# NVlabs/FoundationPose

Hardware: NVIDIA H100
Metric: pose-hypotheses/sec at 640x480 RGB-D, 252 hyp, 5 refine iters (higher is better)
Workload: dtype f16

## Files before the change

foundationpose_b200/csrc/fp_gemm.cu:

```cuda
#include "fp_gemm.cuh"

#include <stdarg.h>
#include <stdlib.h>
#include <string.h>

#include <mutex>
#include <vector>

#include "fp_common.cuh"
#include "fp_wgmma.cuh"

namespace fp {

static std::atomic<unsigned long long> g_launch_count{0};
static thread_local bool t_capturing = false;
void note_launches(int n) {
  if (!t_capturing) g_launch_count.fetch_add((unsigned long long)n, std::memory_order_relaxed);
}
unsigned long long launch_count() { return g_launch_count.load(std::memory_order_relaxed); }
void set_capturing(bool on) { t_capturing = on; }

std::atomic<bool> g_prof_on{false};
static std::mutex g_prof_mu;

struct ProfRec {
  cudaEvent_t e0, e1;
  double work;
  int kind;
};
static std::vector<ProfRec> g_prof_recs;

void prof_mark_begin(int kind, double work, cudaStream_t stream) {
  if (!g_prof_on) return;
  ProfRec r;
  r.kind = kind;
  r.work = work;
  cudaEventCreate(&r.e0);
  cudaEventCreate(&r.e1);
  cudaEventRecord(r.e0, stream);
  std::lock_guard<std::mutex> lk(g_prof_mu);
  g_prof_recs.push_back(r);
}
void prof_mark_end(cudaStream_t stream) {
  if (!g_prof_on) return;
  std::lock_guard<std::mutex> lk(g_prof_mu);
  if (g_prof_recs.empty()) return;
  cudaEventRecord(g_prof_recs.back().e1, stream);
}
int prof_collect(int kind, double* total_ms, double* total_work, int* launches) {
  FP_CUDA_OK(cudaDeviceSynchronize());
  std::lock_guard<std::mutex> lk(g_prof_mu);
  double ms = 0, work = 0;
  int n = 0;
  std::vector<ProfRec> keep;
  for (auto& r : g_prof_recs) {
    if (r.kind != kind) {
      keep.push_back(r);
      continue;
    }
    float t = 0.f;
    cudaEventElapsedTime(&t, r.e0, r.e1);
    ms += t;
    work += r.work;
    ++n;
    cudaEventDestroy(r.e0);
    cudaEventDestroy(r.e1);
  }
  g_prof_recs.swap(keep);
  *total_ms = ms;
  *total_work = work;
  *launches = n;
  return 0;
}

static thread_local char t_last_error[1024] = "";
void set_last_error(const char* fmt, ...) {
  va_list ap;
  va_start(ap, fmt);
  vsnprintf(t_last_error, sizeof(t_last_error), fmt, ap);
  va_end(ap);
}
const char* get_last_error() { return t_last_error; }

static thread_local int t_pdl_skip = 0;
void pdl_skip_next() { t_pdl_skip = 1; }

bool pdl_enabled() {
  if (t_pdl_skip) {
    t_pdl_skip = 0;
    return false;
  }
  static int on = -1;
  if (on < 0) {
    const char* e = getenv("FPOSE_PDL");
    on = (e && e[0] == '0') ? 0 : 1;
  }
  return on != 0;
}

struct GemmParams {
  int lg_bw, lg_bh;
  int bw, bh, bn;
  int tiles_w, tiles_h, tiles_n, n_tiles_n, total_tiles;
  int num_kb, chunks_per_tap;
  int dim_w, dim_h, dim_n;
  short tap_off[9][5];
  int Ho, Wo, n_img, Cout;
  const float* bias;
  int has_res;
  int odim_h, odim_n;
  int out_split;
  const float* post_add;
  int relu;
  double alg_flops;
};

constexpr int kBlockM = 128;
constexpr int kBlockK = 64;
constexpr int kABytes = kBlockM * kBlockK * 2;
constexpr int kTileThreads = 384;
constexpr int kSlabBytes = kBlockM * 64 * 2;
constexpr int kSmemOptIn = 232448;

constexpr int kWideSlabs = 2;
constexpr int kWideProducerRegs = 40;
constexpr int kWideConsumerRegs = 232;
template <int BN>
struct TileCfg {
  static constexpr int kBBytes = BN * kBlockK * 2;
  static constexpr int kStageBytes = kABytes + kBBytes;
  static constexpr int kSlabs = BN > 128 ? kWideSlabs : BN / 64;
  static constexpr int kPasses = BN / 64 / kSlabs;
  static constexpr int kStagingBytes = kSlabs * kSlabBytes;
  static constexpr int kRing = kSmemOptIn - kStagingBytes - 1024  - 256 ;
  static constexpr int kStages = (kRing / kStageBytes) > 8 ? 8 : (kRing / kStageBytes);
  static constexpr int kSmemBytes = kStages * kStageBytes + kStagingBytes + 1024 + 256;
  static_assert(kSmemBytes <= kSmemOptIn, "tile configuration exceeds the 227 KB opt-in shared memory");
  static_assert(kPasses * kSlabs * 64 == BN, "the epilogue passes must cover the tile's channels");
};

template <int BN>
__global__ void __launch_bounds__(kTileThreads, 1)
    gemm_tile_kernel(const __grid_constant__ CUtensorMap map_a, const __grid_constant__ CUtensorMap map_b,
                     const __grid_constant__ CUtensorMap map_out, const __grid_constant__ CUtensorMap map_res,
                     const __grid_constant__ GemmParams p) {
  using Cfg = TileCfg<BN>;
  constexpr int S = Cfg::kStages;
  constexpr int NSLAB = Cfg::kSlabs;
  constexpr int JP = BN / 8 / Cfg::kPasses;
  extern __shared__ uint8_t smem_raw[];
  uint8_t* smem = reinterpret_cast<uint8_t*>((reinterpret_cast<uintptr_t>(smem_raw) + 1023) & ~uintptr_t(1023));
  uint8_t* staging = smem + S * Cfg::kStageBytes;
  uint64_t* bars = reinterpret_cast<uint64_t*>(staging + Cfg::kStagingBytes);
  uint64_t* full = bars;
  uint64_t* empty = bars + S;
  uint64_t* res_full = bars + 2 * S;

  const int m_tiles = p.tiles_w * p.tiles_h * p.tiles_n;
  const int total = m_tiles * p.n_tiles_n;

  if (threadIdx.x == 0) {
    tma_prefetch_desc(&map_a);
    tma_prefetch_desc(&map_b);
    tma_prefetch_desc(&map_out);
    if (p.has_res) tma_prefetch_desc(&map_res);
    for (int s = 0; s < S; ++s) {
      mbar_init(&full[s], 1);
      mbar_init(&empty[s], 256);
    }
    mbar_init(res_full, 1);
    mbar_fence_init();
  }
  __syncthreads();
  pdl_trigger();
  pdl_wait();

  auto decode = [&](int t, int& n_tile, int& tw, int& th, int& tn) {
    n_tile = t % p.n_tiles_n;
    const int m_tile = t / p.n_tiles_n;
    tw = m_tile % p.tiles_w;
    th = (m_tile / p.tiles_w) % p.tiles_h;
    tn = m_tile / (p.tiles_w * p.tiles_h);
  };

  if (threadIdx.x < 128) {
    if constexpr (BN > 128) regs_release<kWideProducerRegs>();
    if (threadIdx.x == 0) {
      int stage = 0, phase = 0;
      for (int t = blockIdx.x; t < total; t += gridDim.x) {
        int n_tile, tw, th, tn;
        decode(t, n_tile, tw, th, tn);
        int base[5] = {0, 0, 0, 0, 0};
        base[p.dim_w] += tw * p.bw;
        if (p.dim_h >= 0) base[p.dim_h] += th * p.bh;
        if (p.dim_n >= 0) base[p.dim_n] += tn * p.bn;
        int tap = 0, chunk = 0;
        for (int kb = 0; kb < p.num_kb; ++kb) {
          mbar_wait(&empty[stage], phase ^ 1);
          uint8_t* sa = smem + stage * Cfg::kStageBytes;
          mbar_expect_tx(&full[stage], Cfg::kStageBytes);
          tma_load_5d(&map_a, &full[stage], sa, base[0] + p.tap_off[tap][0] + chunk * kBlockK, base[1] + p.tap_off[tap][1],
                      base[2] + p.tap_off[tap][2], base[3] + p.tap_off[tap][3], base[4] + p.tap_off[tap][4]);
          tma_load_2d(&map_b, &full[stage], sa + kABytes, kb * kBlockK, n_tile * BN);
          if (++chunk == p.chunks_per_tap) {
            chunk = 0;
            ++tap;
          }
          if (++stage == S) {
            stage = 0;
            phase ^= 1;
          }
        }
      }
    }
    return;
  }

  if constexpr (BN > 128) regs_acquire<kWideConsumerRegs>();
  const int ct = threadIdx.x - 128;
  const int cw = ct >> 7;
  const int lane = threadIdx.x & 31;
  const int r0 = 64 * cw + 16 * ((ct >> 5) & 3) + (lane >> 2);
  const int cq = 2 * (lane & 3);
  const bool leader = (ct == 0);
  float acc[BN / 2];
#pragma unroll
  for (int i = 0; i < BN / 2; ++i) acc[i] = 0.f;
  int stage = 0, phase = 0, it = 0;
  for (int t = blockIdx.x; t < total; t += gridDim.x, ++it) {
    int n_tile, tw, th, tn;
    decode(t, n_tile, tw, th, tn);
    const int n0 = tn * p.bn;
    int n_o0 = n0, coff = 0;
    if (p.out_split > 0) {
      n_o0 = n0 % p.out_split;
      coff = (n0 / p.out_split) * p.Cout;
    }
    int oc[5] = {0, 0, 0, 0, 0}, rc[5] = {0, 0, 0, 0, 0};
    oc[1] = rc[1] = tw * p.bw;
    if (p.odim_h >= 0) oc[p.odim_h] = rc[p.odim_h] = th * p.bh;
    if (p.odim_n >= 0) {
      oc[p.odim_n] = n_o0;
      rc[p.odim_n] = n0;
    }
    if (leader) asm volatile("cp.async.bulk.wait_group.read 0;" ::: "memory");
    asm volatile("bar.sync 1, 256;" ::: "memory");
    if (leader && p.has_res) {
      mbar_expect_tx(res_full, NSLAB * kSlabBytes);
      for (int s = 0; s < NSLAB; ++s)
        tma_load_5d(&map_res, res_full, staging + s * kSlabBytes, n_tile * BN + s * 64, rc[1], rc[2], rc[3], rc[4]);
    }

    int prev = -1;
    for (int kb = 0; kb < p.num_kb; ++kb) {
      mbar_wait(&full[stage], phase);
      const uint32_t sa = smem_u32(smem + stage * Cfg::kStageBytes);
      const uint64_t da = gmma_desc_sw128(sa + (uint32_t)cw * 8192u);
      const uint64_t db = gmma_desc_sw128(sa + kABytes);
      wgmma_fence();
#pragma unroll
      for (int k = 0; k < kBlockK / 16; ++k)
        Wgmma<BN>::ss(acc, da + (uint64_t)(2 * k), db + (uint64_t)(2 * k), (kb > 0 || k > 0) ? 1u : 0u);
      wgmma_commit();
      if (prev >= 0) {
        wgmma_wait<1>();
        mbar_arrive(&empty[prev]);
      }
      prev = stage;
      if (++stage == S) {
        stage = 0;
        phase ^= 1;
      }
    }
    wgmma_wait<0>();
    fence_regs(acc);
    if (prev >= 0) mbar_arrive(&empty[prev]);

    const float* bias = p.bias + n_tile * BN;
    const float* pap[2] = {nullptr, nullptr};
    if (p.post_add) {
#pragma unroll
      for (int h = 0; h < 2; ++h) {
        const int row = r0 + 8 * h;
        const int jj = row & (p.bw - 1), ii = (row >> p.lg_bw) & (p.bh - 1);
        const int i = th * p.bh + ii, j = min(tw * p.bw + jj, p.Wo - 1);
        pap[h] = p.post_add + (size_t)(i * p.Wo + j) * p.Cout + n_tile * BN;
      }
    }
#pragma unroll
    for (int ps = 0; ps < Cfg::kPasses; ++ps) {
      const int c0 = n_tile * BN + ps * NSLAB * 64;
      if (ps > 0) {
        if (leader) asm volatile("cp.async.bulk.wait_group.read 0;" ::: "memory");
        asm volatile("bar.sync 1, 256;" ::: "memory");
        if (leader && p.has_res) {
          mbar_expect_tx(res_full, NSLAB * kSlabBytes);
          for (int s = 0; s < NSLAB; ++s)
            tma_load_5d(&map_res, res_full, staging + s * kSlabBytes, c0 + s * 64, rc[1], rc[2], rc[3], rc[4]);
        }
      }
      if (p.has_res) mbar_wait(res_full, (uint32_t)((it * Cfg::kPasses + ps) & 1));
#pragma unroll
      for (int jl = 0; jl < JP; ++jl) {
        const int j = ps * JP + jl;
        const int col = 8 * j + cq;
        const float2 b = __ldg(reinterpret_cast<const float2*>(bias + col));
        uint8_t* slab = staging + (jl >> 3) * kSlabBytes;
#pragma unroll
        for (int h = 0; h < 2; ++h) {
          const int row = r0 + 8 * h;
          uint32_t* cell = reinterpret_cast<uint32_t*>(slab + row * 128 + ((((uint32_t)j & 7u) ^ (uint32_t)(row & 7)) << 4) + cq * 2);
          float a0 = acc[4 * j + 2 * h] + b.x, a1 = acc[4 * j + 2 * h + 1] + b.y;
          if (p.has_res) {
            const float2 r = __half22float2(*reinterpret_cast<const __half2*>(cell));
            a0 += r.x;
            a1 += r.y;
          }
          if (p.relu) {
            a0 = fmaxf(a0, 0.f);
            a1 = fmaxf(a1, 0.f);
          }
          if (pap[h]) {
            const float2 pe = __ldg(reinterpret_cast<const float2*>(pap[h] + col));
            a0 += pe.x;
            a1 += pe.y;
          }
          *cell = pack_half2(a0, a1);
        }
      }
      asm volatile("fence.proxy.async.shared::cta;" ::: "memory");
      asm volatile("bar.sync 1, 256;" ::: "memory");
      if (leader) {
        for (int s = 0; s < NSLAB; ++s)
          tma_store_5d(&map_out, staging + s * kSlabBytes, coff + c0 + s * 64, oc[1], oc[2], oc[3], oc[4]);
        asm volatile("cp.async.bulk.commit_group;" ::: "memory");
      }
    }
  }
  if (leader) asm volatile("cp.async.bulk.wait_group 0;" ::: "memory");
}

static int g_num_sms = 0;

typedef CUresult (*EncodeTiledFn)(CUtensorMap*, CUtensorMapDataType, cuuint32_t, void*, const cuuint64_t*,
                                  const cuuint64_t*, const cuuint32_t*, const cuuint32_t*,
                                  CUtensorMapInterleave, CUtensorMapSwizzle, CUtensorMapL2promotion,
                                  CUtensorMapFloatOOBfill);

static EncodeTiledFn get_encode_fn() {
  static EncodeTiledFn fn = nullptr;
  static std::once_flag once;
  std::call_once(once, [] {
    void* p = nullptr;
    cudaDriverEntryPointQueryResult qres;
    if (cudaGetDriverEntryPoint("cuTensorMapEncodeTiled", &p, cudaEnableDefault, &qres) == cudaSuccess &&
        qres == cudaDriverEntryPointSuccess)
      fn = reinterpret_cast<EncodeTiledFn>(p);
  });
  return fn;
}

static int encode_map(CUtensorMap* map, const void* base, int rank, const uint64_t* dims,
                      const uint64_t* strides_bytes , const uint32_t* box, bool swizzle128 = true) {
  EncodeTiledFn fn = get_encode_fn();
  FP_REQUIRE(fn != nullptr, "cuTensorMapEncodeTiled entry point not available (no CUDA driver?)");
  cuuint64_t gdim[5];
  cuuint64_t gstr[4];
  cuuint32_t bdim[5];
  cuuint32_t estr[5];
  for (int i = 0; i < rank; ++i) {
    gdim[i] = dims[i];
    bdim[i] = box[i];
    estr[i] = 1;
  }
  for (int i = 0; i < rank - 1; ++i) gstr[i] = strides_bytes[i];
  CUresult r = fn(map, CU_TENSOR_MAP_DATA_TYPE_FLOAT16, (cuuint32_t)rank, const_cast<void*>(base), gdim, gstr,
                  bdim, estr, CU_TENSOR_MAP_INTERLEAVE_NONE, swizzle128 ? CU_TENSOR_MAP_SWIZZLE_128B : CU_TENSOR_MAP_SWIZZLE_NONE,
                  CU_TENSOR_MAP_L2_PROMOTION_L2_256B, CU_TENSOR_MAP_FLOAT_OOB_FILL_NONE);
  FP_REQUIRE(r == CUDA_SUCCESS,
             "cuTensorMapEncodeTiled failed (%d): rank %d dims [%llu %llu %llu %llu %llu] box [%u %u %u %u %u]",
             (int)r, rank, (unsigned long long)dims[0], (unsigned long long)(rank > 1 ? dims[1] : 0),
             (unsigned long long)(rank > 2 ? dims[2] : 0), (unsigned long long)(rank > 3 ? dims[3] : 0),
             (unsigned long long)(rank > 4 ? dims[4] : 0), box[0], rank > 1 ? box[1] : 0, rank > 2 ? box[2] : 0,
             rank > 3 ? box[3] : 0, rank > 4 ? box[4] : 0);
  return 0;
}

int encode_map_f16(CUtensorMap* map, const void* base, int rank, const uint64_t* dims, const uint64_t* strides_bytes,
                   const uint32_t* box) {
  return encode_map(map, base, rank, dims, strides_bytes, box);
}
int encode_map_f16_linear(CUtensorMap* map, const void* base, int rank, const uint64_t* dims,
                          const uint64_t* strides_bytes, const uint32_t* box) {
  return encode_map(map, base, rank, dims, strides_bytes, box, false);
}
int num_sms() {
  if (g_num_sms == 0) {
    int dev = 0;
    if (cudaGetDevice(&dev) != cudaSuccess) return 0;
    if (cudaDeviceGetAttribute(&g_num_sms, cudaDevAttrMultiProcessorCount, dev) != cudaSuccess) return 0;
  }
  return g_num_sms;
}

static int ilog2(int v) {
  int l = 0;
  while ((1 << l) < v) ++l;
  return l;
}

template <int BN>
static int launch_bn(const CUtensorMap& ma, const CUtensorMap& mb, const CUtensorMap& mo, const CUtensorMap& mr,
                     const GemmParams& p, cudaStream_t stream) {
  using Cfg = TileCfg<BN>;
  static std::atomic<unsigned long long> attr_mask{0};
  if (!device_bit_test(attr_mask)) {
    FP_CUDA_OK(cudaFuncSetAttribute(gemm_tile_kernel<BN>, cudaFuncAttributeMaxDynamicSharedMemorySize, Cfg::kSmemBytes));
    device_bit_set(attr_mask);
  }
  const int sms = num_sms();
  FP_REQUIRE(sms > 0, "no CUDA device");
  const int grid = p.total_tiles < sms ? p.total_tiles : sms;
  prof_mark_begin(0, p.alg_flops, stream);
  FP_CUDA_OK(launch_pdl(gemm_tile_kernel<BN>, dim3(grid), dim3(kTileThreads), Cfg::kSmemBytes, stream, 1, ma, mb, mo, mr, p));
  prof_mark_end(stream);
  note_launches(1);
  FP_CUDA_OK(cudaGetLastError());
  return 0;
}

int stem_conv_launch(const GemmLayer& L, cudaStream_t stream);

static int gemm_layer_plan(const GemmLayer& L, cudaStream_t stream, int* tile_n) {
  if (L.kind == LK_CONV7_S2) {
    if (tile_n) {
      *tile_n = 64;
      return 0;
    }
    return stem_conv_launch(L, stream);
  }
  GemmParams p;
  memset(&p, 0, sizeof(p));
  CUtensorMap ma, mb;
  const uint64_t E = 2;
  int Ho, Wo, taps, ktot;
  int BN;
  uint64_t dims[5], str[4];
  uint32_t box[5];

  switch (L.kind) {
    case LK_LINEAR: {
      FP_REQUIRE(L.Cin % 64 == 0, "LINEAR: K=%d not a multiple of 64", L.Cin);
      Ho = 1;
      Wo = L.Win;
      taps = 1;
      p.chunks_per_tap = L.Cin / 64;
      p.bw = 128; p.bh = 1; p.bn = 1;
      p.dim_w = 1; p.dim_h = -1; p.dim_n = -1;
      dims[0] = L.Cin; dims[1] = L.Win; dims[2] = 1; dims[3] = 1; dims[4] = 1;
      str[0] = L.Cin * E; str[1] = str[0] * L.Win; str[2] = str[1]; str[3] = str[1];
      box[0] = 64; box[1] = 128; box[2] = 1; box[3] = 1; box[4] = 1;
      p.tiles_w = (L.Win + 127) / 128; p.tiles_h = 1; p.tiles_n = 1;
      break;
    }
    case LK_CONV3_S1: {
      FP_REQUIRE(L.Cin % 64 == 0, "CONV3_S1: Cin=%d not a multiple of 64", L.Cin);
      Ho = L.Hin; Wo = L.Win;
      taps = 9;
      p.chunks_per_tap = L.Cin / 64;
      if (Wo % 8 == 0 && Ho % 8 == 0) { p.bw = 8; p.bh = 8; p.bn = 2; }
      else if (Wo % 4 == 0 && Ho % 4 == 0) { p.bw = 4; p.bh = 4; p.bn = 8; }
      else FP_REQUIRE(false, "CONV3_S1: unsupported spatial size %dx%d", Ho, Wo);
      const uint64_t sw_ = (uint64_t)L.Cin * E, sh_ = sw_ * L.Win, sn_ = sh_ * L.Hin;
      p.dim_w = 1; p.dim_h = 2; p.dim_n = 3;
      dims[0] = L.Cin; dims[1] = L.Win; dims[2] = L.Hin; dims[3] = L.n_img; dims[4] = 1;
      str[0] = sw_; str[1] = sh_; str[2] = sn_; str[3] = sn_ * L.n_img;
      box[0] = 64; box[1] = p.bw; box[2] = p.bh; box[3] = p.bn; box[4] = 1;
      for (int r = 0; r < 3; ++r)
        for (int s = 0; s < 3; ++s) {
          p.tap_off[r * 3 + s][1] = (short)(s - 1);
          p.tap_off[r * 3 + s][2] = (short)(r - 1);
        }
      p.tiles_w = Wo / p.bw; p.tiles_h = Ho / p.bh; p.tiles_n = (L.n_img + p.bn - 1) / p.bn;
      break;
    }
    case LK_CONV3_S2: {
      FP_REQUIRE(L.Cin % 64 == 0, "CONV3_S2: Cin=%d not a multiple of 64", L.Cin);
      FP_REQUIRE(L.Hin % 2 == 0 && L.Win % 2 == 0, "CONV3_S2: odd input size");
      Ho = L.Hin / 2; Wo = L.Win / 2;
      taps = 9;
      p.chunks_per_tap = L.Cin / 64;
      if (Wo % 8 == 0 && Ho % 8 == 0) { p.bw = 8; p.bh = 8; p.bn = 2; }
      else if (Wo % 4 == 0 && Ho % 4 == 0) { p.bw = 4; p.bh = 4; p.bn = 8; }
      else FP_REQUIRE(false, "CONV3_S2: unsupported output size %dx%d", Ho, Wo);
      p.dim_w = 1; p.dim_h = 3; p.dim_n = 4;
      dims[0] = 2 * L.Cin; dims[1] = Wo; dims[2] = 2; dims[3] = Ho; dims[4] = L.n_img;
      str[0] = 2 * L.Cin * E; str[1] = (uint64_t)L.Win * L.Cin * E; str[2] = 2 * str[1];
      str[3] = (uint64_t)L.Hin * L.Win * L.Cin * E;
      box[0] = 64; box[1] = p.bw; box[2] = 1; box[3] = p.bh; box[4] = p.bn;
      for (int r = 0; r < 3; ++r)
        for (int s = 0; s < 3; ++s) {
          const int t = r * 3 + s;
          p.tap_off[t][0] = (short)((s == 1 ? 0 : 1) * L.Cin);
          p.tap_off[t][1] = (short)(s == 0 ? -1 : 0);
          p.tap_off[t][2] = (short)(r == 1 ? 0 : 1);
          p.tap_off[t][3] = (short)(r == 0 ? -1 : 0);
        }
      p.tiles_w = Wo / p.bw; p.tiles_h = Ho / p.bh; p.tiles_n = (L.n_img + p.bn - 1) / p.bn;
      break;
    }
    default:
      FP_REQUIRE(false, "unknown layer kind %d", L.kind);
  }
  ktot = taps * L.Cin;
  p.num_kb = ktot / 64;
  p.lg_bw = ilog2(p.bw);
  p.lg_bh = ilog2(p.bh);

  constexpr int kWideMinWaves = 8;
  constexpr int kWideMinKBlocks = 16;
  const int m_tiles = p.tiles_w * p.tiles_h * p.tiles_n;
  if (L.Cout % 256 == 0 && p.num_kb >= kWideMinKBlocks) {
    const int sms = num_sms();
    FP_REQUIRE(sms > 0, "no CUDA device");
    BN = (long long)m_tiles * (L.Cout / 256) >= (long long)kWideMinWaves * sms ? 256 : 128;
  } else if (L.Cout % 128 == 0) BN = 128;
  else if (L.Cout % 64 == 0) BN = 64;
  else FP_REQUIRE(false, "Cout=%d must be a multiple of 64", L.Cout);
  p.n_tiles_n = L.Cout / BN;
  p.total_tiles = p.tiles_w * p.tiles_h * p.tiles_n * p.n_tiles_n;
  p.Ho = Ho; p.Wo = Wo; p.n_img = L.n_img; p.Cout = L.Cout;
  p.bias = L.bias;
  p.has_res = L.res != nullptr;
  p.out_split = L.out_split;
  p.post_add = L.post_add;
  p.relu = L.relu;
  {
    const double k_real = (double)taps * L.Cin;
    p.alg_flops = 2.0 * (double)L.n_img * Ho * Wo * L.Cout * k_real;
  }
  FP_REQUIRE(L.out_ld % 8 == 0 && (!L.res || L.res_ld % 8 == 0), "out_ld / res_ld must be multiples of 8");
  FP_REQUIRE(L.out_split == 0 || L.out_split % p.bn == 0,
             "out_split=%d must be a multiple of the tile's image count %d (pad the A/B batch boundary)", L.out_split,
             p.bn);
  if (tile_n) {
    *tile_n = BN;
    return 0;
  }
  if (p.total_tiles == 0) return 0;

  int rc = encode_map(&ma, L.in, 5, dims, str, box);
  if (rc) return rc;
  uint64_t wd[2] = {(uint64_t)ktot, (uint64_t)L.Cout};
  uint64_t ws[1] = {(uint64_t)ktot * E};
  uint32_t wb[2] = {64, (uint32_t)BN};
  rc = encode_map(&mb, L.w, 2, wd, ws, wb);
  if (rc) return rc;
  CUtensorMap mo, mr;
  {
    uint64_t od[5], os[4];
    uint32_t ob[5];
    const bool lin = (L.kind == LK_LINEAR);
    const int n_out = L.out_split > 0 ? (L.n_img - L.out_split) : L.n_img;
    FP_REQUIRE(n_out > 0, "out_split=%d leaves no output images (n_img=%d)", L.out_split, L.n_img);
    auto fill = [&](int ld, int nimg) {
      const uint64_t sw_ = (uint64_t)ld * E, sh_ = sw_ * Wo, sn_ = sh_ * Ho;
      od[0] = (uint64_t)ld;
      ob[0] = 64;
      od[4] = 1;
      ob[4] = 1;
      if (lin) {
        od[1] = (uint64_t)Wo; od[2] = 1; od[3] = 1;
        os[0] = sw_; os[1] = sh_; os[2] = sh_; os[3] = sh_;
        ob[1] = (uint32_t)p.bw; ob[2] = 1; ob[3] = 1;
      } else {
        od[1] = (uint64_t)Wo; od[2] = (uint64_t)Ho; od[3] = (uint64_t)nimg;
        os[0] = sw_; os[1] = sh_; os[2] = sn_; os[3] = sn_ * nimg;
        ob[1] = (uint32_t)p.bw; ob[2] = (uint32_t)p.bh; ob[3] = (uint32_t)p.bn;
      }
    };
    p.odim_h = lin ? -1 : 2;
    p.odim_n = lin ? -1 : 3;
    fill(L.out_ld, n_out);
    rc = encode_map(&mo, L.out, 5, od, os, ob);
    if (rc) return rc;
    if (L.res) {
      fill(L.res_ld, L.n_img);
      rc = encode_map(&mr, L.res, 5, od, os, ob);
      if (rc) return rc;
    } else {
      mr = mo;
    }
  }
  if (BN == 256) return launch_bn<256>(ma, mb, mo, mr, p, stream);
  return BN == 128 ? launch_bn<128>(ma, mb, mo, mr, p, stream) : launch_bn<64>(ma, mb, mo, mr, p, stream);
}

int gemm_layer_launch(const GemmLayer& L, cudaStream_t stream) { return gemm_layer_plan(L, stream, nullptr); }

int gemm_layer_tile_n(const GemmLayer& L, int* tile_n) { return gemm_layer_plan(L, nullptr, tile_n); }

}
```

Baseline: 3542.

## Pipeline GEMM epilogue per 64-channel batch with alternating staging slabs

Restructures the GEMM tile epilogue so wide tiles (BN>128) process output in 64-channel batches that alternate between two staging slabs. Each slab gets its own residual mbarrier, so the next residual TMA load and the previous TMA store overlap with compute on the current batch. The post-add loads for the first batch are issued before the final wgmma wait, and bias and residual reads are batched ahead of use to hide latency. This adds barriers and register pressure (the pe buffer holds 16 float2 per thread), and the phase and wait_group logic is more intricate.

```diff
diff --git a/foundationpose_b200/csrc/fp_gemm.cu b/foundationpose_b200/csrc/fp_gemm.cu
--- a/foundationpose_b200/csrc/fp_gemm.cu
+++ b/foundationpose_b200/csrc/fp_gemm.cu
@@ -129,14 +129,16 @@
 struct TileCfg {
   static constexpr int kBBytes = BN * kBlockK * 2;
   static constexpr int kStageBytes = kABytes + kBBytes;
-  static constexpr int kSlabs = BN > 128 ? kWideSlabs : BN / 64;
-  static constexpr int kPasses = BN / 64 / kSlabs;
+  static constexpr int kBatches = BN / 64;
+  static constexpr bool kAlternate = BN > 128;
+  static constexpr int kSlabs = kAlternate ? kWideSlabs : kBatches;
   static constexpr int kStagingBytes = kSlabs * kSlabBytes;
   static constexpr int kRing = kSmemOptIn - kStagingBytes - 1024  - 256 ;
   static constexpr int kStages = (kRing / kStageBytes) > 8 ? 8 : (kRing / kStageBytes);
   static constexpr int kSmemBytes = kStages * kStageBytes + kStagingBytes + 1024 + 256;
   static_assert(kSmemBytes <= kSmemOptIn, "tile configuration exceeds the 227 KB opt-in shared memory");
-  static_assert(kPasses * kSlabs * 64 == BN, "the epilogue passes must cover the tile's channels");
+  static_assert((2 * kStages + kSlabs) * 8 <= 256, "the mbarriers must fit their 256 bytes");
+  static_assert(kBatches % kSlabs == 0, "every slab must take the same number of batches per tile");
 };
 
 template <int BN>
@@ -147,9 +149,10 @@
   using Cfg = TileCfg<BN>;
   constexpr int S = Cfg::kStages;
   constexpr int NSLAB = Cfg::kSlabs;
-  constexpr int JP = BN / 8 / Cfg::kPasses;
+  constexpr int NB = Cfg::kBatches;
+  constexpr bool kAlt = Cfg::kAlternate;
   extern __shared__ uint8_t smem_raw[];
-  uint8_t* smem = reinterpret_cast<uint8_t*>((reinterpret_cast<uintptr_t>(smem_raw) + 1023) & ~uintptr_t(1023));
+  uint8_t* smem = smem_raw + ((1024u - (smem_u32(smem_raw) & 1023u)) & 1023u);
   uint8_t* staging = smem + S * Cfg::kStageBytes;
   uint64_t* bars = reinterpret_cast<uint64_t*>(staging + Cfg::kStagingBytes);
   uint64_t* full = bars;
@@ -168,7 +171,7 @@
       mbar_init(&full[s], 1);
       mbar_init(&empty[s], 256);
     }
-    mbar_init(res_full, 1);
+    for (int s = 0; s < (kAlt ? NSLAB : 1); ++s) mbar_init(&res_full[s], 1);
     mbar_fence_init();
   }
   __syncthreads();
@@ -246,9 +249,11 @@
     if (leader) asm volatile("cp.async.bulk.wait_group.read 0;" ::: "memory");
     asm volatile("bar.sync 1, 256;" ::: "memory");
     if (leader && p.has_res) {
-      mbar_expect_tx(res_full, NSLAB * kSlabBytes);
-      for (int s = 0; s < NSLAB; ++s)
-        tma_load_5d(&map_res, res_full, staging + s * kSlabBytes, n_tile * BN + s * 64, rc[1], rc[2], rc[3], rc[4]);
+      for (int s = 0; s < NSLAB; ++s) {
+        uint64_t* rb = &res_full[kAlt ? s : 0];
+        if (kAlt || s == 0) mbar_expect_tx(rb, kAlt ? kSlabBytes : NSLAB * kSlabBytes);
+        tma_load_5d(&map_res, rb, staging + s * kSlabBytes, n_tile * BN + s * 64, rc[1], rc[2], rc[3], rc[4]);
+      }
     }
 
     int prev = -1;
@@ -272,10 +277,6 @@
         phase ^= 1;
       }
     }
-    wgmma_wait<0>();
-    fence_regs(acc);
-    if (prev >= 0) mbar_arrive(&empty[prev]);
-
     const float* bias = p.bias + n_tile * BN;
     const float* pap[2] = {nullptr, nullptr};
     if (p.post_add) {
@@ -287,53 +288,84 @@
         pap[h] = p.post_add + (size_t)(i * p.Wo + j) * p.Cout + n_tile * BN;
       }
     }
-#pragma unroll
-    for (int ps = 0; ps < Cfg::kPasses; ++ps) {
-      const int c0 = n_tile * BN + ps * NSLAB * 64;
-      if (ps > 0) {
-        if (leader) asm volatile("cp.async.bulk.wait_group.read 0;" ::: "memory");
+    float2 pe[8][2];
+    auto load_pe = [&](int b) {
+#pragma unroll
+      for (int jl = 0; jl < 8; ++jl)
+#pragma unroll
+        for (int h = 0; h < 2; ++h) pe[jl][h] = __ldg(reinterpret_cast<const float2*>(pap[h] + 64 * b + 8 * jl + cq));
+    };
+    if (p.post_add) load_pe(0);
+    wgmma_wait<0>();
+    fence_regs(acc);
+    if (prev >= 0) mbar_arrive(&empty[prev]);
+
+#pragma unroll
+    for (int b = 0; b < NB; ++b) {
+      const int s = kAlt ? (b & 1) : b;
+      uint8_t* slab = staging + s * kSlabBytes;
+      if (kAlt && p.has_res && b > 0 && b + 1 < NB) {
+        if (leader) {
+          asm volatile("cp.async.bulk.wait_group.read 0;" ::: "memory");
+          uint64_t* rb = &res_full[(b + 1) & 1];
+          mbar_expect_tx(rb, kSlabBytes);
+          tma_load_5d(&map_res, rb, staging + ((b + 1) & 1) * kSlabBytes, n_tile * BN + (b + 1) * 64, rc[1], rc[2],
+                      rc[3], rc[4]);
+        }
+      }
+      if (p.has_res && (kAlt || b == 0))
+        mbar_wait(&res_full[kAlt ? s : 0], (uint32_t)((it * (NB / NSLAB) + b / NSLAB) & 1));
+#pragma unroll
+      for (int jh = 0; jh < 8; jh += 4) {
+        float2 bb[4];
+        __half2 rv[4][2];
+#pragma unroll
+        for (int jl = 0; jl < 4; ++jl) {
+          bb[jl] = __ldg(reinterpret_cast<const float2*>(bias + 64 * b + 8 * (jh + jl) + cq));
+          if (p.has_res) {
+#pragma unroll
+            for (int h = 0; h < 2; ++h) {
+              const int row = r0 + 8 * h;
+              rv[jl][h] = *reinterpret_cast<const __half2*>(slab + row * 128 + (((uint32_t)(jh + jl) ^ (uint32_t)(row & 7)) << 4) + cq * 2);
+            }
+          }
+        }
+#pragma unroll
+        for (int jl = 0; jl < 4; ++jl) {
+          const int j = 8 * b + jh + jl;
+#pragma unroll
+          for (int h = 0; h < 2; ++h) {
+            const int row = r0 + 8 * h;
+            uint32_t* cell = reinterpret_cast<uint32_t*>(slab + row * 128 + (((uint32_t)(jh + jl) ^ (uint32_t)(row & 7)) << 4) + cq * 2);
+            float a0 = acc[4 * j + 2 * h] + bb[jl].x, a1 = acc[4 * j + 2 * h + 1] + bb[jl].y;
+            if (p.has_res) {
+              const float2 r = __half22float2(rv[jl][h]);
+              a0 += r.x;
+              a1 += r.y;
+            }
+            if (p.relu) {
+              a0 = fmaxf(a0, 0.f);
+              a1 = fmaxf(a1, 0.f);
+            }
+            if (p.post_add) {
+              a0 += pe[jh + jl][h].x;
+              a1 += pe[jh + jl][h].y;
+            }
+            *cell = pack_half2(a0, a1);
+          }
+        }
+      }
+      if (p.post_add && b + 1 < NB) load_pe(b + 1);
+      if (kAlt || b == NB - 1) {
+        asm volatile("fence.proxy.async.shared::cta;" ::: "memory");
+        if (kAlt && leader) asm volatile("cp.async.bulk.wait_group.read 0;" ::: "memory");
         asm volatile("bar.sync 1, 256;" ::: "memory");
-        if (leader && p.has_res) {
-          mbar_expect_tx(res_full, NSLAB * kSlabBytes);
-          for (int s = 0; s < NSLAB; ++s)
-            tma_load_5d(&map_res, res_full, staging + s * kSlabBytes, c0 + s * 64, rc[1], rc[2], rc[3], rc[4]);
+        if (leader) {
+          for (int q = kAlt ? s : 0; q < (kAlt ? s + 1 : NSLAB); ++q)
+            tma_store_5d(&map_out, staging + q * kSlabBytes, coff + n_tile * BN + (kAlt ? 64 * b : 64 * q), oc[1],
+                         oc[2], oc[3], oc[4]);
+          asm volatile("cp.async.bulk.commit_group;" ::: "memory");
         }
-      }
-      if (p.has_res) mbar_wait(res_full, (uint32_t)((it * Cfg::kPasses + ps) & 1));
-#pragma unroll
-      for (int jl = 0; jl < JP; ++jl) {
-        const int j = ps * JP + jl;
-        const int col = 8 * j + cq;
-        const float2 b = __ldg(reinterpret_cast<const float2*>(bias + col));
-        uint8_t* slab = staging + (jl >> 3) * kSlabBytes;
-#pragma unroll
-        for (int h = 0; h < 2; ++h) {
-          const int row = r0 + 8 * h;
-          uint32_t* cell = reinterpret_cast<uint32_t*>(slab + row * 128 + ((((uint32_t)j & 7u) ^ (uint32_t)(row & 7)) << 4) + cq * 2);
-          float a0 = acc[4 * j + 2 * h] + b.x, a1 = acc[4 * j + 2 * h + 1] + b.y;
-          if (p.has_res) {
-            const float2 r = __half22float2(*reinterpret_cast<const __half2*>(cell));
-            a0 += r.x;
-            a1 += r.y;
-          }
-          if (p.relu) {
-            a0 = fmaxf(a0, 0.f);
-            a1 = fmaxf(a1, 0.f);
-          }
-          if (pap[h]) {
-            const float2 pe = __ldg(reinterpret_cast<const float2*>(pap[h] + col));
-            a0 += pe.x;
-            a1 += pe.y;
-          }
-          *cell = pack_half2(a0, a1);
-        }
-      }
-      asm volatile("fence.proxy.async.shared::cta;" ::: "memory");
-      asm volatile("bar.sync 1, 256;" ::: "memory");
-      if (leader) {
-        for (int s = 0; s < NSLAB; ++s)
-          tma_store_5d(&map_out, staging + s * kSlabBytes, coff + c0 + s * 64, oc[1], oc[2], oc[3], oc[4]);
-        asm volatile("cp.async.bulk.commit_group;" ::: "memory");
       }
     }
   }
```

After: 3657 (median of 6 runs). +3.2%, better.
